# IDEA-CCNL/Fengshenbang-LM

Measured on AMD Instinct MI355X. Metric: tokens/sec Ziya-LLaMA-13B ZeRO-3, higher is better.
Workload: dtype bf16; 1 GPU; model=Ziya-LLaMA-13B, global_batch=16, micro_batch=16, seq_len=2048, parallelism=zero3_dp1, activation_checkpointing=True, ckpt_skip_interval=4

## Files before the change

fengshen_amd/models/layers.py:

```python
from __future__ import annotations

import math
from typing import Callable, List, Optional

import torch
import torch.nn as nn
import torch.nn.init as init

from fengshen_amd.ops import functional as F_ops
from fengshen_amd.parallel import groups
from fengshen_amd.parallel.layers import (
    ColumnParallelLinear,
    RowParallelLinear,
    _init_partition,
    divide,
)
from fengshen_amd.parallel.mappings import (
    copy_to_tensor_model_parallel_region,
    gather_from_tensor_model_parallel_region,
)


def init_normal(std: float) -> Callable:
    def fn(tensor):
# ... 219 lines not shown

    def __init__(self, hidden_size: int, intermediate_size: Optional[int] = None,
                 multiple_of: int = 256, init_method=None,
                 output_init_method=None, dtype=None,
                 reduce_output: bool = True):
        super().__init__()
        self.reduce_output = reduce_output
        if intermediate_size is None:
            intermediate_size = int(2 * (4 * hidden_size) / 3)
            intermediate_size = multiple_of * (
                (intermediate_size + multiple_of - 1) // multiple_of)
        self.intermediate_size = intermediate_size
        init_method = init_method or init.xavier_normal_
        self.gate_up_proj = MergedColumnParallelLinear(
            hidden_size, [intermediate_size, intermediate_size], bias=False,
            init_method=init_method, dtype=dtype)
        self.down_proj = RowParallelLinear(
            intermediate_size, hidden_size, bias=False, input_is_parallel=True,
            init_method=output_init_method or init_method, dtype=dtype,
            reduce_output=reduce_output)

    def forward(self, x):
        packed = self.gate_up_proj(x)
        h = F_ops.swiglu(packed)
        return self.down_proj(h)


class ParallelTransformerLayer(nn.Module):

    def __init__(self, hidden_size: int, num_heads: int, *, causal: bool,
                 norm: str = "layernorm", norm_eps: float = 1e-5,
                 mlp_type: str = "gelu", ffn_hidden_size=None,
                 rotary: bool = False, rope_base: float = 10000.0,
                 max_positions: int = 4096,
                 attention_dropout: float = 0.0, hidden_dropout: float = 0.0,
                 bias: bool = True, init_method=None, output_init_method=None,
                 dtype=None, layer_idx: int = 0,
                 parallel_residual: bool = False):
        super().__init__()
        self.parallel_residual = parallel_residual
        self.input_norm = get_norm(norm, hidden_size, norm_eps, dtype)
        self.attention = ParallelAttention(
            hidden_size, num_heads, causal=causal, rotary=rotary,
            rope_base=rope_base, max_positions=max_positions,
            attention_dropout=attention_dropout, hidden_dropout=hidden_dropout,
            bias=bias, init_method=init_method,
            output_init_method=output_init_method, dtype=dtype,
            layer_idx=layer_idx, reduce_output=not parallel_residual)
        self.post_attention_norm = get_norm(norm, hidden_size, norm_eps, dtype)
        if mlp_type == "swiglu":
            self.mlp = LLaMAParallelMLP(
                hidden_size, ffn_hidden_size, init_method=init_method,
                output_init_method=output_init_method, dtype=dtype,
                reduce_output=not parallel_residual)
        else:
            self.mlp = ParallelMLP(
                hidden_size, ffn_hidden_size, bias=bias, init_method=init_method,
                output_init_method=output_init_method, dtype=dtype,
                reduce_output=not parallel_residual)
        self.hidden_dropout = hidden_dropout

    @staticmethod
    def _split_partial(out):
        if isinstance(out, tuple):
            return out[0], out[1]
        return out, None

    def forward(self, x, attention_mask=None, cache=None):
        if self.parallel_residual:
            from fengshen_amd.parallel.mappings import (
                reduce_from_tensor_model_parallel_region)
            ap, ab = self._split_partial(self.attention(
                self.input_norm(x), attention_mask=attention_mask,
                cache=cache))
            mp, mb = self._split_partial(
                self.mlp(self.post_attention_norm(x)))
            total = reduce_from_tensor_model_parallel_region(ap + mp)
            bias = None
            if ab is not None or mb is not None:
                bias = (ab if ab is not None else 0)                     + (mb if mb is not None else 0)
            return F_ops.bias_dropout_add(total, bias, x,
                                          self.hidden_dropout,
                                          self.training)
        residual = x
        h = self.input_norm(x)
        attn_out = self.attention(h, attention_mask=attention_mask, cache=cache)
        x = F_ops.bias_dropout_add(attn_out, None, residual,
                                   self.hidden_dropout, self.training)
        residual = x
        h = self.post_attention_norm(x)
        mlp_out = self.mlp(h)
        x = F_ops.bias_dropout_add(mlp_out, None, residual,
                                   self.hidden_dropout, self.training)
        return x


def parallel_lm_logits(hidden: torch.Tensor, word_embeddings_weight: torch.Tensor,
                       parallel_output: bool = True):
    input_parallel = copy_to_tensor_model_parallel_region(hidden)
    logits_parallel = torch.nn.functional.linear(
        input_parallel, word_embeddings_weight)
    if parallel_output:
        return logits_parallel
    return gather_from_tensor_model_parallel_region(logits_parallel)


class SinusoidalPositionalEmbedding(nn.Module):

    def __init__(self, dim: int, base: float = 10000.0):
        super().__init__()
        self.dim = dim
        self.base = base

    def forward(self, positions: torch.Tensor) -> torch.Tensor:
        half = self.dim // 2
        inv = 1.0 / (self.base ** (torch.arange(
            half, device=positions.device, dtype=torch.float32) / half))
        ang = positions.float()[..., None] * inv
        return torch.cat([ang.sin(), ang.cos()], dim=-1)


class AliBi(nn.Module):

    def __init__(self, num_heads: int, mp_size: int = 1, mp_rank: int = 0):
        super().__init__()
        self.num_heads = num_heads
        slopes = torch.tensor(self._slopes(num_heads))
        per = num_heads // mp_size
        self.register_buffer("slopes", slopes[mp_rank * per:(mp_rank + 1) * per],
                             persistent=False)
        self._cache = None

    @staticmethod
    def _slopes(n: int):
        def pow2(n):
            start = 2.0 ** (-(2.0 ** -(math.log2(n) - 3)))
            return [start * (start ** i) for i in range(n)]
        if math.log2(n).is_integer():
            return pow2(n)
        closest = 2 ** math.floor(math.log2(n))
        return pow2(closest) + AliBi._slopes(2 * closest)[0::2][: n - closest]

    def forward(self, sq: int, sk: int, device, dtype):
        if (self._cache is None or self._cache.shape[-1] < sk
                or self._cache.device != device):
            pos = torch.arange(sk, device=device, dtype=torch.float32)
            self._cache = self.slopes.to(device)[:, None, None] * \
                (pos[None, None, :] - pos[None, :, None])
        bias = self._cache[:, :sq, :sk] if self._cache.shape[1] >= sq else \
            self._cache[:, -sq:, :sk]
        return bias.to(dtype)


class SoftEmbedding(nn.Module):

    def __init__(self, wte: nn.Module, n_tokens: int = 10,
                 init_range: float = 0.5):
        super().__init__()
        self.wte = wte
        self.n_tokens = n_tokens
        dim = wte.weight.shape[1]
        self.soft_prompt = nn.Parameter(
            torch.empty(n_tokens, dim).uniform_(-init_range, init_range))

    def forward(self, input_ids: torch.Tensor) -> torch.Tensor:
        emb = self.wte(input_ids)
        b = emb.shape[0]
        prompt = self.soft_prompt.unsqueeze(0).expand(b, -1, -1).to(emb.dtype)
        return torch.cat([prompt, emb], dim=1)


class SpatialGatingUnit(nn.Module):

# ... 70 lines not shown
```

fengshen_amd/ops/build.py:

```python
from __future__ import annotations

import glob
import os
import shutil
import sys

_OPS_DIR = os.path.dirname(os.path.abspath(__file__))
_CSRC = os.path.join(_OPS_DIR, "csrc")
_BUILD_DIR = os.path.join(_OPS_DIR, "_build")
_TARGET = os.path.join(_OPS_DIR, "_C.so")


def sources():
    srcs = [os.path.join(_CSRC, "bindings.cpp"),
            os.path.join(_CSRC, "kernels.hip")]
    fa = os.path.join(_CSRC, "flash_attn.hip")
    if os.path.exists(fa):
        srcs.append(fa)
    return srcs


def needs_rebuild() -> bool:
    if not os.path.exists(_TARGET):
        return True
    t = os.path.getmtime(_TARGET)
    deps = sources() + glob.glob(os.path.join(_CSRC, "*.h"))
    return any(os.path.getmtime(s) > t for s in deps)


def build(force: bool = False, verbose: bool = True) -> str:
    os.environ.setdefault("PYTORCH_ROCM_ARCH", "gfx950")
    if not force and not needs_rebuild():
        if verbose:
            print(f"[fengshen_amd.ops.build] up to date: {_TARGET}")
        return _TARGET
    from torch.utils.cpp_extension import load

    os.makedirs(_BUILD_DIR, exist_ok=True)
    load(
        name="_C",
        sources=sources(),
        extra_cflags=["-O3", "-std=c++17"],
        extra_cuda_cflags=["-O3", "-std=c++17", "--offload-arch=gfx950",
                           "-ffast-math"],
        build_directory=_BUILD_DIR,
        verbose=verbose,
        is_python_module=False,
        keep_intermediates=True,
    )
    built = os.path.join(_BUILD_DIR, "_C.so")
    if not os.path.exists(built):
        cands = glob.glob(os.path.join(_BUILD_DIR, "_C*.so"))
        if not cands:
            raise RuntimeError(f"extension build produced no .so in {_BUILD_DIR}")
        built = cands[0]
    shutil.copy2(built, _TARGET)
    if verbose:
        print(f"[fengshen_amd.ops.build] built {_TARGET}")
    build_data_helpers(force=force, verbose=verbose)
    return _TARGET


_DATA_DIR = os.path.normpath(os.path.join(_OPS_DIR, "..", "data"))
_HELPERS_SRC = os.path.join(_DATA_DIR, "csrc", "helpers.cpp")
_HELPERS_TARGET = os.path.join(_DATA_DIR, "_helpers.so")


def build_data_helpers(force: bool = False, verbose: bool = True) -> str:
    if not force and os.path.exists(_HELPERS_TARGET) and \
            os.path.getmtime(_HELPERS_TARGET) > os.path.getmtime(_HELPERS_SRC):
        return _HELPERS_TARGET
    import subprocess
    import sysconfig

    import pybind11

    cmd = [
        "c++", "-O3", "-std=c++17", "-shared", "-fPIC",
        f"-I{pybind11.get_include()}",
        f"-I{sysconfig.get_paths()['include']}",
        _HELPERS_SRC, "-o", _HELPERS_TARGET,
    ]
    subprocess.check_call(cmd)
    if verbose:
        print(f"[fengshen_amd.ops.build] built {_HELPERS_TARGET}")
    return _HELPERS_TARGET


if __name__ == "__main__":
    build(force="--force" in sys.argv)
```

fengshen_amd/ops/csrc/bindings.cpp:

```cpp
#include <torch/extension.h>

#include <hip/hip_runtime.h>
#include <c10/hip/HIPStream.h>

#include <vector>

enum FsDtype { FS_F32 = 0, FS_BF16 = 1, FS_F16 = 2 };

static int fs_dtype(const at::Tensor& t) {
  switch (t.scalar_type()) {
    case at::kFloat: return FS_F32;
    case at::kBFloat16: return FS_BF16;
    case at::kHalf: return FS_F16;
    default: TORCH_CHECK(false, "unsupported dtype ", t.scalar_type());
  }
}

static hipStream_t cur_stream() {
  return c10::hip::getCurrentHIPStream().stream();
}

extern "C" {
void fs_rms_norm_fwd(const void*, const void*, void*, float*, int, int, float,
                     int, hipStream_t);
void fs_rms_norm_bwd(const void*, const void*, const void*, const float*,
                     void*, float*, int, int, int, hipStream_t);
void fs_layer_norm_fwd(const void*, const void*, const void*, void*, float*,
                       float*, int, int, float, int, hipStream_t);
void fs_layer_norm_bwd(const void*, const void*, const void*, const float*,
                       const float*, void*, float*, float*, int, int, int,
                       hipStream_t);
void fs_scaled_softmax_fwd(const void*, const unsigned char*, void*, float,
                           int, int, int, int, int, int, int, int,
                           hipStream_t);
void fs_scaled_softmax_bwd(const void*, const void*, void*, float, int, int,
                           int, hipStream_t);
void fs_rope(const void*, void*, const float*, const float*, long, int, int,
             int, int, int, hipStream_t);
void fs_swiglu_fwd(const void*, void*, long, int, int, hipStream_t);
void fs_swiglu_bwd(const void*, const void*, void*, long, int, int,
                   hipStream_t);
void fs_bias_gelu(const void*, const void*, const void*, void*, long, int, int,
                  int, hipStream_t);
void fs_fused_adamw(float*, const void*, float*, float*, void*, long, float,
                    float, float, float, float, int, int, int, hipStream_t);
void fs_flash_attn_fwd(const void*, const void*, const void*, void*, float*,
                       const int*, int, int, int, int, int, int, float,
                       float, unsigned long long, hipStream_t);
void fs_flash_attn_bwd(const void*, const void*, const void*, const void*,
                       const void*, const float*, void*, void*, void*, float*,
                       const int*, int, int, int, int, int, int, float,
                       float, unsigned long long, hipStream_t);
void fs_bf16_gemv(const void*, const void*, void*, int, int, int,
                  hipStream_t);
void fs_add_rms_norm(const void*, const void*, const void*, void*, void*,
                     int, int, float, hipStream_t);
void fs_decode_attn(const void*, void*, void*, const float*, const float*,
                    const void*, void*, int, int, int, int, float, int,
                    hipStream_t);
void fs_w8_gemv(const void*, const float*, const void*, void*, int, int, int,
                hipStream_t);
void fs_vocab_ce_fwd(const void*, const long*, float*, float*, float*,
                     long, int, int, int, hipStream_t);
void fs_vocab_ce_bwd(const void*, const long*, const float*, const float*,
                     const float*, void*, long, int, int, int, hipStream_t);
void fs_flash_attn_fwd_v3(const void*, const void*, const void*, void*,
                          float*, const int*, int, int, int, int, int, float,
                          float, unsigned long long, hipStream_t);
void fs_flash_attn_bwd_v3(const void*, const void*, const void*, const void*,
                          const void*, const float*, void*, void*, void*,
                          float*, const int*, int, int, int, int, int, float,
                          float, unsigned long long, hipStream_t);
void fs_flash_attn_fwd_v3_strided(const void*, const void*, const void*,
                                  void*, float*, const int*, const long*,
                                  const long*, int, int, int, int, int, float,
                                  float, unsigned long long, hipStream_t);
void fs_flash_attn_bwd_v3_strided(const void*, const void*, const void*,
                                  const void*, const void*, const float*,
                                  void*, void*, void*, float*, const int*,
                                  const long*, const long*, const long*,
                                  const long*, int, int, int, int, int, float,
                                  float, unsigned long long, hipStream_t);
void fs_rope_inplace(void*, void*, const float*, const float*, int, int, int,
                     int, long, long, long, int, int, int, hipStream_t);
}

static std::vector<at::Tensor> rms_norm_fwd(at::Tensor x, at::Tensor w,
                                            double eps) {
  TORCH_CHECK(x.is_contiguous() && w.is_contiguous());
  const int H = x.size(-1);
  TORCH_CHECK(H % 8 == 0, "hidden must be divisible by 8");
  const long rows = x.numel() / H;
  auto out = at::empty_like(x);
  auto invrms = at::empty({rows}, x.options().dtype(at::kFloat));
  fs_rms_norm_fwd(x.data_ptr(), w.data_ptr(), out.data_ptr(),
                  invrms.data_ptr<float>(), (int)rows, H, (float)eps,
                  fs_dtype(x), cur_stream());
  return {out, invrms};
}

static std::vector<at::Tensor> rms_norm_bwd(at::Tensor gy, at::Tensor x,
                                            at::Tensor w, at::Tensor invrms) {
  const int H = x.size(-1);
  const long rows = x.numel() / H;
  auto gx = at::empty_like(x);
  auto gw32 = at::zeros({H}, x.options().dtype(at::kFloat));
  fs_rms_norm_bwd(gy.data_ptr(), x.data_ptr(), w.data_ptr(),
                  invrms.data_ptr<float>(), gx.data_ptr(),
                  gw32.data_ptr<float>(), (int)rows, H, fs_dtype(x),
                  cur_stream());
  return {gx, gw32.to(w.scalar_type())};
}

static std::vector<at::Tensor> layer_norm_fwd(at::Tensor x, at::Tensor w,
                                              c10::optional<at::Tensor> b,
                                              double eps) {
  TORCH_CHECK(x.is_contiguous());
  const int H = x.size(-1);
  TORCH_CHECK(H % 8 == 0, "hidden must be divisible by 8");
  const long rows = x.numel() / H;
  auto out = at::empty_like(x);
  auto mean = at::empty({rows}, x.options().dtype(at::kFloat));
  auto invstd = at::empty({rows}, x.options().dtype(at::kFloat));
  fs_layer_norm_fwd(x.data_ptr(), w.data_ptr(),
                    b.has_value() ? b->data_ptr() : nullptr, out.data_ptr(),
                    mean.data_ptr<float>(), invstd.data_ptr<float>(),
                    (int)rows, H, (float)eps, fs_dtype(x), cur_stream());
  return {out, mean, invstd};
}

static std::vector<at::Tensor> layer_norm_bwd(at::Tensor gy, at::Tensor x,
                                              at::Tensor w, at::Tensor mean,
                                              at::Tensor invstd) {
  const int H = x.size(-1);
  const long rows = x.numel() / H;
  auto gx = at::empty_like(x);
  auto gw32 = at::zeros({H}, x.options().dtype(at::kFloat));
  auto gb32 = at::zeros({H}, x.options().dtype(at::kFloat));
  fs_layer_norm_bwd(gy.data_ptr(), x.data_ptr(), w.data_ptr(),
                    mean.data_ptr<float>(), invstd.data_ptr<float>(),
                    gx.data_ptr(), gw32.data_ptr<float>(),
                    gb32.data_ptr<float>(), (int)rows, H, fs_dtype(x),
                    cur_stream());
  return {gx, gw32.to(w.scalar_type()), gb32.to(w.scalar_type())};
}

static at::Tensor scaled_masked_softmax_fwd(at::Tensor x,
                                            c10::optional<at::Tensor> mask,
                                            double scale) {
  TORCH_CHECK(x.dim() == 4 && x.is_contiguous());
  const int sk = x.size(3), sq = x.size(2), np = x.size(1), b = x.size(0);
  auto out = at::empty_like(x);
  const unsigned char* mp = nullptr;
  at::Tensor m8;
  int mb = 1, mode = 0, mask_sq = 1;
  if (mask.has_value()) {
    m8 = mask->to(at::kByte).contiguous();
    TORCH_CHECK(m8.dim() == 4 && m8.size(3) == sk &&
                    (m8.size(2) == sq || m8.size(2) == 1),
                "mask must be [mb,1,sq|1,sk]");
    mb = m8.size(0);
    mask_sq = m8.size(2);
    TORCH_CHECK(mb == 1 || mb == b, "mask batch must be 1 or b");
    mp = m8.data_ptr<unsigned char>();
    mode = 1;
  }
  fs_scaled_softmax_fwd(x.data_ptr(), mp, out.data_ptr(), (float)scale,
                        b * np * sq, sk, sq, np, mb, mask_sq, mode,
                        fs_dtype(x), cur_stream());
  return out;
}

static at::Tensor scaled_causal_softmax_fwd(at::Tensor x, double scale) {
  TORCH_CHECK(x.dim() == 3 && x.is_contiguous());
  const int sk = x.size(2), sq = x.size(1), ab = x.size(0);
  TORCH_CHECK(sq == sk, "causal softmax needs sq == sk");
  auto out = at::empty_like(x);
  fs_scaled_softmax_fwd(x.data_ptr(), nullptr, out.data_ptr(), (float)scale,
                        ab * sq, sk, sq, 1, 1, sq, 2, fs_dtype(x),
                        cur_stream());
  return out;
}

static at::Tensor scaled_softmax_bwd(at::Tensor gy, at::Tensor y,
                                     double scale) {
  TORCH_CHECK(gy.is_contiguous() && y.is_contiguous());
  const int sk = y.size(-1);
  const long rows = y.numel() / sk;
  auto gx = at::empty_like(y);
  fs_scaled_softmax_bwd(gy.data_ptr(), y.data_ptr(), gx.data_ptr(),
                        (float)scale, (int)rows, sk, fs_dtype(y),
                        cur_stream());
  return gx;
}
// ... 346 lines not shown
  mod.def("add_rms_norm", &add_rms_norm);
  mod.def("flash_attn_fwd", &flash_attn_fwd);
  mod.def("vocab_ce_fwd", [](at::Tensor logits2d, at::Tensor targets,
                             int64_t vstart, int64_t vend) {
    TORCH_CHECK(logits2d.is_contiguous() && logits2d.dim() == 2
                && logits2d.scalar_type() == at::kBFloat16);
    TORCH_CHECK(targets.scalar_type() == at::kLong
                && targets.is_contiguous());
    const long n = logits2d.size(0);
    const int w = logits2d.size(1);
    TORCH_CHECK(w % 8 == 0, "vocab shard must be divisible by 8");
    auto opts = logits2d.options().dtype(at::kFloat);
    auto m = at::empty({n}, opts);
    auto z = at::empty({n}, opts);
    auto pred = at::empty({n}, opts);
    fs_vocab_ce_fwd(logits2d.data_ptr(), targets.data_ptr<long>(),
                    m.data_ptr<float>(), z.data_ptr<float>(),
                    pred.data_ptr<float>(), n, w, (int)vstart, (int)vend,
                    cur_stream());
    return std::vector<at::Tensor>{m, z, pred};
  });
  mod.def("vocab_ce_bwd", [](at::Tensor logits2d, at::Tensor targets,
                             at::Tensor m, at::Tensor z, at::Tensor gout,
                             int64_t vstart, int64_t vend) {
    const long n = logits2d.size(0);
    const int w = logits2d.size(1);
    auto dl = at::empty_like(logits2d);
    fs_vocab_ce_bwd(logits2d.data_ptr(), targets.data_ptr<long>(),
                    m.data_ptr<float>(), z.data_ptr<float>(),
                    gout.contiguous().data_ptr<float>(), dl.data_ptr(), n, w,
                    (int)vstart, (int)vend, cur_stream());
    return dl;
  });
  mod.def("flash_attn_bwd_v3", [](at::Tensor q, at::Tensor k, at::Tensor v,
                                  at::Tensor o, at::Tensor dout,
                                  at::Tensor lse, double scale, bool causal,
                                  c10::optional<at::Tensor> klens,
                                  double drop_p, int64_t seed) {
    const int b = q.size(0), h = q.size(1), s = q.size(2), d = q.size(3);
    TORCH_CHECK((d == 128 || d == 96 || d == 64) && s % 64 == 0);
    const int* klp = nullptr;
    if (klens.has_value()) klp = klens->data_ptr<int>();
    auto dq = at::empty_like(q);
    auto dk = at::empty_like(k);
    auto dv = at::empty_like(v);
    auto delta = at::empty({b, h, s}, q.options().dtype(at::kFloat));
    fs_flash_attn_bwd_v3(q.data_ptr(), k.data_ptr(), v.data_ptr(),
                         o.data_ptr(), dout.contiguous().data_ptr(),
                         lse.data_ptr<float>(), dq.data_ptr(), dk.data_ptr(),
                         dv.data_ptr(), delta.data_ptr<float>(), klp, b, h,
                         s, d, causal ? 1 : 0, (float)scale, (float)drop_p,
                         (unsigned long long)seed, cur_stream());
    return std::vector<at::Tensor>{dq, dk, dv};
  });
  mod.def("flash_attn_fwd_v3", [](at::Tensor q, at::Tensor k, at::Tensor v,
                                  double scale, bool causal,
                                  c10::optional<at::Tensor> klens,
                                  double drop_p, int64_t seed) {
    TORCH_CHECK(q.is_contiguous() && k.is_contiguous() && v.is_contiguous());
    TORCH_CHECK(q.scalar_type() == at::kBFloat16);
    const int b = q.size(0), h = q.size(1), s = q.size(2), d = q.size(3);
    TORCH_CHECK((d == 128 || d == 96 || d == 64) && s % 64 == 0 && s >= 64);
    TORCH_CHECK(k.size(2) == s, "v3 is self-attention (sq == sk)");
    const int* klp = nullptr;
    if (klens.has_value()) {
      TORCH_CHECK(klens->scalar_type() == at::kInt
                  && klens->numel() == b && klens->is_contiguous());
      klp = klens->data_ptr<int>();
    }
    auto o = at::empty_like(q);
    auto lse = at::empty({b, h, s}, q.options().dtype(at::kFloat));
    fs_flash_attn_fwd_v3(q.data_ptr(), k.data_ptr(), v.data_ptr(),
                         o.data_ptr(), lse.data_ptr<float>(), klp, b, h, s,
                         d, causal ? 1 : 0, (float)scale, (float)drop_p,
                         (unsigned long long)seed, cur_stream());
    return std::vector<at::Tensor>{o, lse};
  });
  mod.def("flash_attn_bwd", &flash_attn_bwd);
  mod.def("flash_attn_fwd_v3_strided", &flash_attn_fwd_v3_strided);
  mod.def("flash_attn_bwd_v3_strided", &flash_attn_bwd_v3_strided);
  mod.def("rope_inplace", &rope_inplace);
  mod.def("rms_norm_fwd", &rms_norm_fwd);
  mod.def("rms_norm_bwd", &rms_norm_bwd);
  mod.def("layer_norm_fwd", &layer_norm_fwd);
  mod.def("layer_norm_bwd", &layer_norm_bwd);
  mod.def("scaled_masked_softmax_fwd", &scaled_masked_softmax_fwd);
  mod.def("scaled_causal_softmax_fwd", &scaled_causal_softmax_fwd);
  mod.def("scaled_softmax_bwd", &scaled_softmax_bwd);
  mod.def("rope_fwd", &rope_fwd);
  mod.def("rope_bwd", &rope_bwd);
  mod.def("swiglu_fwd", &swiglu_fwd);
  mod.def("swiglu_bwd", &swiglu_bwd);
  mod.def("bias_gelu_fwd", &bias_gelu_fwd);
  mod.def("bias_gelu_bwd", &bias_gelu_bwd);
  mod.def("fused_adamw", &fused_adamw);
}
```

fengshen_amd/ops/functional.py:

```python
from __future__ import annotations

import math
from typing import Optional

import torch

from fengshen_amd.ops import use_hip, get_ext


def eager_scaled_masked_softmax(x: torch.Tensor, mask: Optional[torch.Tensor],
                                scale: float) -> torch.Tensor:
    y = x.float() * scale
    if mask is not None:
        y = y.masked_fill(mask.bool(), -10000.0)
    return torch.softmax(y, dim=-1).to(x.dtype)


def eager_scaled_causal_softmax(x: torch.Tensor, scale: float) -> torch.Tensor:
    sq, sk = x.shape[-2], x.shape[-1]
    y = x.float() * scale
    causal = torch.ones(sq, sk, dtype=torch.bool, device=x.device).triu(1)
    y = y.masked_fill(causal, -10000.0)
    return torch.softmax(y, dim=-1).to(x.dtype)


class _ScaledMaskedSoftmax(torch.autograd.Function):
    @staticmethod
    def forward(ctx, x, mask, scale):
        if use_hip(x):
            out = get_ext().scaled_masked_softmax_fwd(x.contiguous(), mask,
                                                      scale)
        else:
            out = eager_scaled_masked_softmax(x, mask, scale)
        ctx.save_for_backward(out)
        ctx.scale = scale
        return out

    @staticmethod
    def backward(ctx, grad_out):
        (out,) = ctx.saved_tensors
        if use_hip(out):
            grad_in = get_ext().scaled_softmax_bwd(grad_out.contiguous(), out,
                                                   ctx.scale)
        else:
            g = grad_out.float() * out.float()
            grad_in = ((g - out.float() * g.sum(dim=-1, keepdim=True))
                       * ctx.scale).to(out.dtype)
        return grad_in, None, None


class _ScaledCausalSoftmax(torch.autograd.Function):
    @staticmethod
    def forward(ctx, x, scale):
        if use_hip(x):
            out = get_ext().scaled_causal_softmax_fwd(x.contiguous(), scale)
        else:
            out = eager_scaled_causal_softmax(x, scale)
        ctx.save_for_backward(out)
        ctx.scale = scale
        return out

    @staticmethod
    def backward(ctx, grad_out):
        (out,) = ctx.saved_tensors
        if use_hip(out):
            grad_in = get_ext().scaled_softmax_bwd(grad_out.contiguous(), out,
                                                   ctx.scale)
        else:
            g = grad_out.float() * out.float()
            grad_in = ((g - out.float() * g.sum(dim=-1, keepdim=True))
                       * ctx.scale).to(out.dtype)
        return grad_in, None


def scaled_masked_softmax(x, mask, scale: float = 1.0):
    return _ScaledMaskedSoftmax.apply(x, mask, scale)


def scaled_causal_softmax(x, scale: float = 1.0):
    return _ScaledCausalSoftmax.apply(x, scale)


def eager_rms_norm(x: torch.Tensor, weight: torch.Tensor, eps: float):
    x32 = x.float()
    var = x32.pow(2).mean(-1, keepdim=True)
    y = x32 * torch.rsqrt(var + eps)
    return (weight.float() * y).to(x.dtype)


class _RMSNorm(torch.autograd.Function):
    @staticmethod
    def forward(ctx, x, weight, eps):
        if use_hip(x):
            x = x.contiguous()
            out, invrms = get_ext().rms_norm_fwd(x, weight, eps)
        else:
            x32 = x.float()
            var = x32.pow(2).mean(-1, keepdim=True)
            invrms = torch.rsqrt(var + eps)
            out = (x32 * invrms * weight.float()).to(x.dtype)
        ctx.save_for_backward(x, weight, invrms)
        return out

    @staticmethod
    def backward(ctx, grad_out):
        x, weight, invrms = ctx.saved_tensors
        if use_hip(x):
            gx, gw = get_ext().rms_norm_bwd(grad_out.contiguous(), x, weight,
                                            invrms)
            return gx, gw, None
        x32 = x.float()
        g32 = grad_out.float()
        w32 = weight.float()
        xhat = x32 * invrms
        gy_w = g32 * w32
        mean_term = (gy_w * xhat).mean(-1, keepdim=True)
        gx = (invrms * (gy_w - xhat * mean_term)).to(x.dtype)
        gw = (g32 * xhat).sum(dim=tuple(range(x.dim() - 1))).to(weight.dtype)
        return gx, gw, None


def rms_norm(x, weight, eps: float = 1e-6):
    return _RMSNorm.apply(x, weight, eps)


def eager_layer_norm(x, weight, bias, eps):
    return torch.nn.functional.layer_norm(
        x.float(), (x.shape[-1],), weight.float(),
        bias.float() if bias is not None else None, eps).to(x.dtype)


class _LayerNorm(torch.autograd.Function):
    @staticmethod
    def forward(ctx, x, weight, bias, eps):
        if use_hip(x):
            x = x.contiguous()
            out, mean, invstd = get_ext().layer_norm_fwd(x, weight, bias, eps)
            ctx.save_for_backward(x, weight, mean, invstd)
            ctx.has_bias = bias is not None
            return out
        ctx.eps = eps
        ctx.fallback = True
        x32 = x.float()
        mean = x32.mean(-1, keepdim=True)
        var = x32.var(-1, unbiased=False, keepdim=True)
        invstd = torch.rsqrt(var + eps)
        out = (x32 - mean) * invstd * weight.float()
        if bias is not None:
            out = out + bias.float()
        ctx.save_for_backward(x, weight, mean, invstd)
        ctx.has_bias = bias is not None
        return out.to(x.dtype)

    @staticmethod
    def backward(ctx, grad_out):
        x, weight, mean, invstd = ctx.saved_tensors
        if use_hip(x):
            gx, gw, gb = get_ext().layer_norm_bwd(
                grad_out.contiguous(), x, weight, mean, invstd)
            return gx, gw, (gb if ctx.has_bias else None), None
        x32 = x.float()
        g32 = grad_out.float()
        w32 = weight.float()
        xhat = (x32 - mean) * invstd
        gy_w = g32 * w32
        n = x.shape[-1]
        gx = (invstd * (gy_w - gy_w.mean(-1, keepdim=True)
                        - xhat * (gy_w * xhat).mean(-1, keepdim=True))).to(x.dtype)
        dims = tuple(range(x.dim() - 1))
        gw = (g32 * xhat).sum(dims).to(weight.dtype)
        gb = g32.sum(dims).to(weight.dtype) if ctx.has_bias else None
        return gx, gw, gb, None


def layer_norm(x, weight, bias=None, eps: float = 1e-5):
    return _LayerNorm.apply(x, weight, bias, eps)


def eager_gelu(x):
    return x * 0.5 * (1.0 + torch.tanh(0.79788456 * x * (1 + 0.044715 * x * x)))


class _BiasGelu(torch.autograd.Function):
    @staticmethod
    def forward(ctx, x, bias):
        ctx.save_for_backward(x, bias)
        if use_hip(x):
            return get_ext().bias_gelu_fwd(x, bias)
        y = x.float() + bias.float()
        return eager_gelu(y).to(x.dtype)

    @staticmethod
    def backward(ctx, grad_out):
        x, bias = ctx.saved_tensors
        if use_hip(x):
            gx = get_ext().bias_gelu_bwd(grad_out.contiguous(), x, bias)
        else:
            y = (x.float() + bias.float())
            t = torch.tanh(0.79788456 * y * (1 + 0.044715 * y * y))
            ff = 0.5 * y * ((1 - t * t) * (0.79788456 + 0.1070322243 * y * y)) \
                + 0.5 * (1 + t)
            gx = (ff * grad_out.float()).to(x.dtype)
        gb = gx.sum(dim=tuple(range(gx.dim() - 1))).to(bias.dtype)
        return gx, gb


# ... 183 lines not shown
```

Measured before the change: 10170 tokens/s.

## Fuse residual add with RMSNorm forward and backward in decoder layers

```diff
diff --git a/fengshen_amd/models/layers.py b/fengshen_amd/models/layers.py
--- a/fengshen_amd/models/layers.py
+++ b/fengshen_amd/models/layers.py
@@ -325,13 +325,25 @@
             return F_ops.bias_dropout_add(total, bias, x,
                                           self.hidden_dropout,
                                           self.training)
+        fused = (isinstance(self.input_norm, RMSNorm)
+                 and isinstance(self.post_attention_norm, RMSNorm)
+                 and (self.hidden_dropout == 0.0 or not self.training))
+        if fused:
+            residual, h = F_ops.residual_rms_norm(
+                x, None, self.input_norm.weight, self.input_norm.eps)
+        else:
+            residual = x
+            h = self.input_norm(x)
+        attn_out = self.attention(h, attention_mask=attention_mask, cache=cache)
+        if fused and torch.is_tensor(attn_out):
+            x, h = F_ops.residual_rms_norm(
+                residual, attn_out, self.post_attention_norm.weight,
+                self.post_attention_norm.eps)
+        else:
+            x = F_ops.bias_dropout_add(attn_out, None, residual,
+                                       self.hidden_dropout, self.training)
+            h = self.post_attention_norm(x)
         residual = x
-        h = self.input_norm(x)
-        attn_out = self.attention(h, attention_mask=attention_mask, cache=cache)
-        x = F_ops.bias_dropout_add(attn_out, None, residual,
-                                   self.hidden_dropout, self.training)
-        residual = x
-        h = self.post_attention_norm(x)
         mlp_out = self.mlp(h)
         x = F_ops.bias_dropout_add(mlp_out, None, residual,
                                    self.hidden_dropout, self.training)
diff --git a/fengshen_amd/ops/build.py b/fengshen_amd/ops/build.py
--- a/fengshen_amd/ops/build.py
+++ b/fengshen_amd/ops/build.py
@@ -13,7 +13,8 @@
 
 def sources():
     srcs = [os.path.join(_CSRC, "bindings.cpp"),
-            os.path.join(_CSRC, "kernels.hip")]
+            os.path.join(_CSRC, "kernels.hip"),
+            os.path.join(_CSRC, "fused_norm.hip")]
     fa = os.path.join(_CSRC, "flash_attn.hip")
     if os.path.exists(fa):
         srcs.append(fa)
diff --git a/fengshen_amd/ops/csrc/bindings.cpp b/fengshen_amd/ops/csrc/bindings.cpp
--- a/fengshen_amd/ops/csrc/bindings.cpp
+++ b/fengshen_amd/ops/csrc/bindings.cpp
@@ -3,6 +3,7 @@
 #include <hip/hip_runtime.h>
 #include <c10/hip/HIPStream.h>
 
+#include <string>
 #include <vector>
 
 enum FsDtype { FS_F32 = 0, FS_BF16 = 1, FS_F16 = 2 };
@@ -83,6 +84,13 @@
                                   float, unsigned long long, hipStream_t);
 void fs_rope_inplace(void*, void*, const float*, const float*, int, int, int,
                      int, long, long, long, int, int, int, hipStream_t);
+int fs_fused_norm_vectors(int);
+int fs_fused_norm_bwd_grid(int, int);
+void fs_res_rms_norm_fwd(const void*, const void*, const void*, void*, void*,
+                         float*, int, int, float, int, hipStream_t);
+void fs_res_rms_norm_bwd(const void*, const void*, const void*, const void*,
+                         const float*, void*, float*, void*, int, int, int,
+                         hipStream_t);
 }
 
 static std::vector<at::Tensor> rms_norm_fwd(at::Tensor x, at::Tensor w,
@@ -110,6 +118,69 @@
                   gw32.data_ptr<float>(), (int)rows, H, fs_dtype(x),
                   cur_stream());
   return {gx, gw32.to(w.scalar_type())};
+}
+
+static std::string fused_norm_branch(int64_t H) {
+  const int nv = fs_fused_norm_vectors((int)H);
+  return nv ? "reg" + std::to_string(nv) : std::string("lds");
+}
+
+static std::vector<at::Tensor> residual_rms_norm_fwd(
+    at::Tensor x, c10::optional<at::Tensor> delta, at::Tensor w, double eps) {
+  TORCH_CHECK(x.is_contiguous() && w.is_contiguous());
+  const int H = x.size(-1);
+  TORCH_CHECK(H % 8 == 0, "hidden must be divisible by 8");
+  TORCH_CHECK(w.numel() == H && w.scalar_type() == x.scalar_type());
+  const bool has_delta = delta.has_value();
+  if (has_delta)
+    TORCH_CHECK(delta->is_contiguous() && delta->sizes() == x.sizes() &&
+                delta->scalar_type() == x.scalar_type());
+  if (fs_fused_norm_vectors(H) == 0) {
+    at::Tensor sum = has_delta ? at::add(x, *delta) : x;
+    auto r = rms_norm_fwd(sum, w, eps);
+    return {sum, r[0], r[1]};
+  }
+  const long rows = x.numel() / H;
+  at::Tensor sum = has_delta ? at::empty_like(x) : x;
+  auto h = at::empty_like(x);
+  auto invrms = at::empty({rows}, x.options().dtype(at::kFloat));
+  fs_res_rms_norm_fwd(x.data_ptr(), has_delta ? delta->data_ptr() : nullptr,
+                      w.data_ptr(), has_delta ? sum.data_ptr() : nullptr,
+                      h.data_ptr(), invrms.data_ptr<float>(), (int)rows, H,
+                      (float)eps, fs_dtype(x), cur_stream());
+  return {sum, h, invrms};
+}
+
+static std::vector<at::Tensor> residual_rms_norm_bwd(
+    at::Tensor g_h, c10::optional<at::Tensor> g_res, at::Tensor x,
+    at::Tensor w, at::Tensor invrms) {
+  TORCH_CHECK(g_h.is_contiguous() && x.is_contiguous() && w.is_contiguous());
+  TORCH_CHECK(g_h.sizes() == x.sizes() &&
+              g_h.scalar_type() == x.scalar_type());
+  const int H = x.size(-1);
+  const long rows = x.numel() / H;
+  TORCH_CHECK(H % 8 == 0, "hidden must be divisible by 8");
+  TORCH_CHECK(invrms.is_contiguous() && invrms.scalar_type() == at::kFloat &&
+              invrms.numel() == rows, "invrms must be ", rows, " floats");
+  TORCH_CHECK(w.numel() == H);
+  const bool has_res = g_res.has_value();
+  if (has_res)
+    TORCH_CHECK(g_res->is_contiguous() && g_res->sizes() == x.sizes() &&
+                g_res->scalar_type() == x.scalar_type());
+  if (fs_fused_norm_vectors(H) == 0) {
+    auto r = rms_norm_bwd(g_h, x, w, invrms);
+    return {has_res ? at::add(r[0], *g_res) : r[0], r[1]};
+  }
+  TORCH_CHECK(w.scalar_type() == x.scalar_type());
+  auto g = at::empty_like(x);
+  auto gw = at::empty_like(w);
+  auto part = at::empty({fs_fused_norm_bwd_grid((int)rows, H), H},
+                        x.options().dtype(at::kFloat));
+  fs_res_rms_norm_bwd(g_h.data_ptr(), has_res ? g_res->data_ptr() : nullptr,
+                      x.data_ptr(), w.data_ptr(), invrms.data_ptr<float>(),
+                      g.data_ptr(), part.data_ptr<float>(), gw.data_ptr(),
+                      (int)rows, H, fs_dtype(x), cur_stream());
+  return {g, gw};
 }
 
 static std::vector<at::Tensor> layer_norm_fwd(at::Tensor x, at::Tensor w,
@@ -622,6 +693,9 @@
   mod.def("rope_inplace", &rope_inplace);
   mod.def("rms_norm_fwd", &rms_norm_fwd);
   mod.def("rms_norm_bwd", &rms_norm_bwd);
+  mod.def("residual_rms_norm_fwd", &residual_rms_norm_fwd);
+  mod.def("residual_rms_norm_bwd", &residual_rms_norm_bwd);
+  mod.def("fused_norm_branch", &fused_norm_branch);
   mod.def("layer_norm_fwd", &layer_norm_fwd);
   mod.def("layer_norm_bwd", &layer_norm_bwd);
   mod.def("scaled_masked_softmax_fwd", &scaled_masked_softmax_fwd);
diff --git a/fengshen_amd/ops/csrc/fused_norm.hip b/fengshen_amd/ops/csrc/fused_norm.hip
--- /dev/null
+++ b/fengshen_amd/ops/csrc/fused_norm.hip
@@ -0,0 +1,351 @@
+
+#include "common.h"
+
+enum FsDtype { FS_F32 = 0, FS_BF16 = 1, FS_F16 = 2 };
+
+namespace {
+
+template <typename T>
+__device__ __forceinline__ float round_to(float v) {
+  return to_f32<T>(from_f32<T>(v));
+}
+
+constexpr int FN_THREADS = 256;
+constexpr int FN_WAVES = FN_THREADS / WAVE_SIZE;
+
+__device__ __forceinline__ float fn_block_sum(float v, float* red) {
+#pragma clang fp reassociate(off)
+  v = wave_reduce_sum(v);
+  if ((threadIdx.x & (WAVE_SIZE - 1)) == 0) red[threadIdx.x / WAVE_SIZE] = v;
+  __syncthreads();
+  const float a = red[0] + red[2];
+  const float b = red[1] + red[3];
+  return a + b;
+}
+
+__device__ __forceinline__ float row_partial(float acc, const float (&a)[8],
+                                             const float (&b)[8]) {
+#pragma clang fp reassociate(off) contract(off)
+  float lo = a[6] * b[6];
+  float hi = a[7] * b[7];
+  lo = __builtin_fmaf(a[2], b[2], lo);
+  hi = __builtin_fmaf(a[3], b[3], hi);
+  lo = __builtin_fmaf(a[4], b[4], lo);
+  hi = __builtin_fmaf(a[5], b[5], hi);
+  lo = __builtin_fmaf(a[0], b[0], lo);
+  hi = __builtin_fmaf(a[1], b[1], hi);
+  const float s = lo + hi;
+  return acc + s;
+}
+
+__device__ __forceinline__ float norm_out(float x, float ir, float w) {
+#pragma clang fp reassociate(off)
+  return (w * ir) * x;
+}
+
+__device__ __forceinline__ float norm_grad(float gyw, float xh, float dot,
+                                           float ir) {
+#pragma clang fp reassociate(off) contract(off)
+  return __builtin_fmaf(-dot, xh, gyw) * ir;
+}
+
+template <typename T>
+__device__ __forceinline__ float add_rounded(float inner, float r) {
+  float t = round_to<T>(inner);
+  if constexpr (sizeof(T) == 4) asm volatile("" : "+v"(t));
+  return t + r;
+}
+
+__device__ __forceinline__ float row_mean(float sum, int H) {
+#pragma clang fp reassociate(off)
+  return sum / H;
+}
+
+__device__ __forceinline__ void zero8(float (&v)[8]) {
+#pragma unroll
+  for (int i = 0; i < 8; ++i) v[i] = 0.f;
+}
+
+template <typename T> struct raw8 { short8_t v; };
+template <> struct raw8<float> { float4_t lo, hi; };
+
+template <typename T>
+__device__ __forceinline__ raw8<T> raw_zero() {
+  raw8<T> r;
+  r.v = short8_t{0, 0, 0, 0, 0, 0, 0, 0};
+  return r;
+}
+template <>
+__device__ __forceinline__ raw8<float> raw_zero<float>() {
+  raw8<float> r;
+  r.lo = float4_t{0.f, 0.f, 0.f, 0.f};
+  r.hi = r.lo;
+  return r;
+}
+
+template <typename T>
+__device__ __forceinline__ raw8<T> raw_load(const T* p) {
+  raw8<T> r;
+  r.v = *reinterpret_cast<const short8_t*>(p);
+  return r;
+}
+template <>
+__device__ __forceinline__ raw8<float> raw_load<float>(const float* p) {
+  raw8<float> r;
+  r.lo = reinterpret_cast<const float4_t*>(p)[0];
+  r.hi = reinterpret_cast<const float4_t*>(p)[1];
+  return r;
+}
+
+template <typename T>
+__device__ __forceinline__ void unpack8(const raw8<T>& r, float (&out)[8]) {
+  load8<T>(reinterpret_cast<const T*>(&r.v), out);
+}
+template <>
+__device__ __forceinline__ void unpack8<float>(const raw8<float>& r,
+                                               float (&out)[8]) {
+#pragma unroll
+  for (int i = 0; i < 4; ++i) { out[i] = r.lo[i]; out[4 + i] = r.hi[i]; }
+}
+
+template <typename T, int V, bool HAS_DELTA>
+__global__ __launch_bounds__(FN_THREADS) void res_rms_norm_fwd_kernel(
+    const T* __restrict__ x, const T* __restrict__ delta,
+    const T* __restrict__ w, T* __restrict__ sum_out, T* __restrict__ h_out,
+    float* __restrict__ invrms, int rows, int H, float eps) {
+  __shared__ float red[2][FN_WAVES];
+  int c[V];
+  bool act[V];
+  raw8<T> wr[V], xr[V], dr[V];
+  int row = blockIdx.x;
+#pragma unroll
+  for (int p = 0; p < V; ++p) {
+    c[p] = (threadIdx.x + p * FN_THREADS) * 8;
+    act[p] = c[p] < H;
+    wr[p] = xr[p] = dr[p] = raw_zero<T>();
+    if (act[p]) {
+      wr[p] = raw_load<T>(w + c[p]);
+      if (row < rows) {
+        xr[p] = raw_load<T>(x + (long)row * H + c[p]);
+        if (HAS_DELTA) dr[p] = raw_load<T>(delta + (long)row * H + c[p]);
+      }
+    }
+  }
+  int buf = 0;
+  for (; row < rows; row += gridDim.x) {
+    float v[V][8];
+#pragma unroll
+    for (int p = 0; p < V; ++p) {
+      unpack8<T>(xr[p], v[p]);
+      if (HAS_DELTA) {
+        float dv[8];
+        unpack8<T>(dr[p], dv);
+#pragma unroll
+        for (int i = 0; i < 8; ++i) v[p][i] = round_to<T>(v[p][i] + dv[i]);
+      }
+    }
+    const int nrow = row + gridDim.x;
+    if (nrow < rows) {
+#pragma unroll
+      for (int p = 0; p < V; ++p)
+        if (act[p]) {
+          xr[p] = raw_load<T>(x + (long)nrow * H + c[p]);
+          if (HAS_DELTA) dr[p] = raw_load<T>(delta + (long)nrow * H + c[p]);
+        }
+    }
+    float ss = 0.f;
+#pragma unroll
+    for (int p = 0; p < V; ++p) {
+      if (HAS_DELTA && act[p]) store8<T>(sum_out + (long)row * H + c[p], v[p]);
+      ss = row_partial(ss, v[p], v[p]);
+    }
+    ss = fn_block_sum(ss, red[buf]);
+    buf ^= 1;
+    const float ir = rsqrtf(ss / H + eps);
+    if (threadIdx.x == 0) invrms[row] = ir;
+#pragma unroll
+    for (int p = 0; p < V; ++p)
+      if (act[p]) {
+        float wv[8], o[8];
+        unpack8<T>(wr[p], wv);
+#pragma unroll
+        for (int i = 0; i < 8; ++i) o[i] = norm_out(v[p][i], ir, wv[i]);
+        store8<T>(h_out + (long)row * H + c[p], o);
+      }
+  }
+}
+
+template <typename T, int V, bool HAS_RES>
+__global__ __launch_bounds__(FN_THREADS) void res_rms_norm_bwd_kernel(
+    const T* __restrict__ gh, const T* __restrict__ gres,
+    const T* __restrict__ x, const T* __restrict__ w,
+    const float* __restrict__ invrms, T* __restrict__ g_out,
+    float* __restrict__ gw_part, int rows, int H) {
+  __shared__ float red[2][FN_WAVES];
+  int c[V];
+  bool act[V];
+  float acc[V][8];
+  raw8<T> wr[V], xr[V], gr[V], rr[V];
+  int row = blockIdx.x;
+#pragma unroll
+  for (int p = 0; p < V; ++p) {
+    c[p] = (threadIdx.x + p * FN_THREADS) * 8;
+    act[p] = c[p] < H;
+    zero8(acc[p]);
+    wr[p] = xr[p] = gr[p] = rr[p] = raw_zero<T>();
+    if (act[p]) {
+      wr[p] = raw_load<T>(w + c[p]);
+      if (row < rows) {
+        xr[p] = raw_load<T>(x + (long)row * H + c[p]);
+        gr[p] = raw_load<T>(gh + (long)row * H + c[p]);
+        if (HAS_RES) rr[p] = raw_load<T>(gres + (long)row * H + c[p]);
+      }
+    }
+  }
+  int buf = 0;
+  for (; row < rows; row += gridDim.x) {
+    const float ir = invrms[row];
+    float xh[V][8], gyw[V][8];
+    raw8<T> rcur[V];
+    float dot = 0.f;
+#pragma unroll
+    for (int p = 0; p < V; ++p) {
+      float xv[8], gv[8], wv[8];
+      unpack8<T>(xr[p], xv);
+      unpack8<T>(gr[p], gv);
+      unpack8<T>(wr[p], wv);
+#pragma unroll
+      for (int i = 0; i < 8; ++i) {
+        xh[p][i] = xv[i] * ir;
+        gyw[p][i] = gv[i] * wv[i];
+        acc[p][i] += gv[i] * xh[p][i];
+      }
+      dot = row_partial(dot, gyw[p], xh[p]);
+      rcur[p] = rr[p];
+    }
+    const int nrow = row + gridDim.x;
+    if (nrow < rows) {
+#pragma unroll
+      for (int p = 0; p < V; ++p)
+        if (act[p]) {
+          xr[p] = raw_load<T>(x + (long)nrow * H + c[p]);
+          gr[p] = raw_load<T>(gh + (long)nrow * H + c[p]);
+          if (HAS_RES) rr[p] = raw_load<T>(gres + (long)nrow * H + c[p]);
+        }
+    }
+    dot = row_mean(fn_block_sum(dot, red[buf]), H);
+    buf ^= 1;
+#pragma unroll
+    for (int p = 0; p < V; ++p)
+      if (act[p]) {
+        float o[8], r[8];
+        unpack8<T>(rcur[p], r);
+#pragma unroll
+        for (int i = 0; i < 8; ++i) {
+          o[i] = norm_grad(gyw[p][i], xh[p][i], dot, ir);
+          if (HAS_RES) o[i] = add_rounded<T>(o[i], r[i]);
+        }
+        store8<T>(g_out + (long)row * H + c[p], o);
+      }
+  }
+#pragma unroll
+  for (int p = 0; p < V; ++p)
+    if (act[p]) {
+      float4_t* q =
+          reinterpret_cast<float4_t*>(gw_part + (long)blockIdx.x * H + c[p]);
+      float4_t lo = {acc[p][0], acc[p][1], acc[p][2], acc[p][3]};
+      float4_t hi = {acc[p][4], acc[p][5], acc[p][6], acc[p][7]};
+      q[0] = lo;
+      q[1] = hi;
+    }
+}
+
+template <typename T>
+__global__ __launch_bounds__(512) void rms_norm_gw_reduce_kernel(
+    const float* __restrict__ part, T* __restrict__ gw, int P, int H) {
+  __shared__ float sm[8][64];
+  const int tx = threadIdx.x & 63;
+  const int ty = threadIdx.x >> 6;
+  const int col = blockIdx.x * 64 + tx;
+  float s = 0.f;
+  if (col < H)
+    for (int p = ty; p < P; p += 8) s += part[(long)p * H + col];
+  sm[ty][tx] = s;
+  __syncthreads();
+  if (ty == 0 && col < H) {
+    float t = 0.f;
+#pragma unroll
+    for (int i = 0; i < 8; ++i) t += sm[i][tx];
+    gw[col] = from_f32<T>(t);
+  }
+}
+
+#define FN_DISPATCH_DTYPE(dtype, T, ...)                      \
+  switch (dtype) {                                            \
+    case FS_F32: { using T = float; __VA_ARGS__; break; }     \
+    case FS_BF16: { using T = bf16_t; __VA_ARGS__; break; }   \
+    case FS_F16: { using T = fp16_t; __VA_ARGS__; break; }    \
+  }
+
+#define FN_DISPATCH_V(nv, V, ...)                             \
+  switch (nv) {                                               \
+    case 1: { constexpr int V = 1; __VA_ARGS__; break; }      \
+    case 2: { constexpr int V = 2; __VA_ARGS__; break; }      \
+    case 3: { constexpr int V = 3; __VA_ARGS__; break; }      \
+    case 4: { constexpr int V = 4; __VA_ARGS__; break; }      \
+  }
+
+#define FN_DISPATCH_BOOL(flag, B, ...)                        \
+  if (flag) { constexpr bool B = true; __VA_ARGS__; }         \
+  else { constexpr bool B = false; __VA_ARGS__; }
+
+}
+
+extern "C" {
+
+int fs_fused_norm_vectors(int H) {
+  if (H % 8 != 0 || H < 256 || H > 8192) return 0;
+  return (H + FN_THREADS * 8 - 1) / (FN_THREADS * 8);
+}
+
+int fs_fused_norm_bwd_grid(int rows, int H) {
+  if (fs_fused_norm_vectors(H) == 0) return 0;
+  const int g = rows < 1024 ? rows : 1024;
+  return g < 1 ? 1 : g;
+}
+
+void fs_res_rms_norm_fwd(const void* x, const void* delta, const void* w,
+                         void* sum_out, void* h_out, float* invrms, int rows,
+                         int H, float eps, int dtype, hipStream_t s) {
+  const int nv = fs_fused_norm_vectors(H);
+  int grid = rows < FS_MAX_BLOCKS ? rows : FS_MAX_BLOCKS;
+  if (grid < 1) grid = 1;
+  FN_DISPATCH_DTYPE(dtype, T,
+    FN_DISPATCH_V(nv, V,
+      FN_DISPATCH_BOOL(delta != nullptr, HD,
+        hipLaunchKernelGGL((res_rms_norm_fwd_kernel<T, V, HD>), dim3(grid),
+                           dim3(FN_THREADS), 0, s, (const T*)x,
+                           (const T*)delta, (const T*)w, (T*)sum_out,
+                           (T*)h_out, invrms, rows, H, eps))));
+}
+
+void fs_res_rms_norm_bwd(const void* gh, const void* gres, const void* x,
+                         const void* w, const float* invrms, void* g_out,
+                         float* gw_part, void* gw, int rows, int H, int dtype,
+                         hipStream_t s) {
+  const int nv = fs_fused_norm_vectors(H);
+  const int grid = fs_fused_norm_bwd_grid(rows, H);
+  FN_DISPATCH_DTYPE(dtype, T,
+    FN_DISPATCH_V(nv, V,
+      FN_DISPATCH_BOOL(gres != nullptr, HR,
+        hipLaunchKernelGGL((res_rms_norm_bwd_kernel<T, V, HR>), dim3(grid),
+                           dim3(FN_THREADS), 0, s, (const T*)gh,
+                           (const T*)gres, (const T*)x, (const T*)w, invrms,
+                           (T*)g_out, gw_part, rows, H))));
+  FN_DISPATCH_DTYPE(dtype, T,
+    hipLaunchKernelGGL((rms_norm_gw_reduce_kernel<T>), dim3((H + 63) / 64),
+                       dim3(512), 0, s, (const float*)gw_part, (T*)gw, grid,
+                       H));
+}
+
+}
diff --git a/fengshen_amd/ops/functional.py b/fengshen_amd/ops/functional.py
--- a/fengshen_amd/ops/functional.py
+++ b/fengshen_amd/ops/functional.py
@@ -1,6 +1,7 @@
 from __future__ import annotations
 
 import math
+import os
 from typing import Optional
 
 import torch
@@ -88,12 +89,33 @@
     return (weight.float() * y).to(x.dtype)
 
 
+def fused_norm_enabled() -> bool:
+    return os.environ.get("FENGSHEN_FUSED_NORM", "1") != "0"
+
+
+def _rms_norm_bwd_eager(g_h, x, weight, invrms):
+    x32 = x.float()
+    g32 = g_h.float()
+    w32 = weight.float()
+    xhat = x32 * invrms
+    gy_w = g32 * w32
+    mean_term = (gy_w * xhat).mean(-1, keepdim=True)
+    gx = (invrms * (gy_w - xhat * mean_term)).to(x.dtype)
+    gw = (g32 * xhat).sum(dim=tuple(range(x.dim() - 1))).to(weight.dtype)
+    return gx, gw
+
+
 class _RMSNorm(torch.autograd.Function):
     @staticmethod
     def forward(ctx, x, weight, eps):
+        ctx.fused = fused_norm_enabled()
         if use_hip(x):
             x = x.contiguous()
-            out, invrms = get_ext().rms_norm_fwd(x, weight, eps)
+            if ctx.fused:
+                _, out, invrms = get_ext().residual_rms_norm_fwd(
+                    x, None, weight, eps)
+            else:
+                out, invrms = get_ext().rms_norm_fwd(x, weight, eps)
         else:
             x32 = x.float()
             var = x32.pow(2).mean(-1, keepdim=True)
@@ -106,22 +128,64 @@
     def backward(ctx, grad_out):
         x, weight, invrms = ctx.saved_tensors
         if use_hip(x):
-            gx, gw = get_ext().rms_norm_bwd(grad_out.contiguous(), x, weight,
-                                            invrms)
+            if ctx.fused:
+                gx, gw = get_ext().residual_rms_norm_bwd(
+                    grad_out.contiguous(), None, x, weight, invrms)
+            else:
+                gx, gw = get_ext().rms_norm_bwd(grad_out.contiguous(), x,
+                                                weight, invrms)
             return gx, gw, None
-        x32 = x.float()
-        g32 = grad_out.float()
-        w32 = weight.float()
-        xhat = x32 * invrms
-        gy_w = g32 * w32
-        mean_term = (gy_w * xhat).mean(-1, keepdim=True)
-        gx = (invrms * (gy_w - xhat * mean_term)).to(x.dtype)
-        gw = (g32 * xhat).sum(dim=tuple(range(x.dim() - 1))).to(weight.dtype)
+        gx, gw = _rms_norm_bwd_eager(grad_out, x, weight, invrms)
         return gx, gw, None
 
 
 def rms_norm(x, weight, eps: float = 1e-6):
     return _RMSNorm.apply(x, weight, eps)
+
+
+class _ResidualRMSNorm(torch.autograd.Function):
+
+    @staticmethod
+    def forward(ctx, x, delta, weight, eps):
+        ctx.set_materialize_grads(False)
+        ctx.has_delta = delta is not None
+        if use_hip(x):
+            xc = x.contiguous()
+            dc = delta.contiguous() if ctx.has_delta else None
+            res, h, invrms = get_ext().residual_rms_norm_fwd(
+                xc, dc, weight, eps)
+            if not ctx.has_delta:
+                res = x
+        else:
+            res = x + delta if ctx.has_delta else x
+            r32 = res.float()
+            invrms = torch.rsqrt(r32.pow(2).mean(-1, keepdim=True) + eps)
+            h = (r32 * invrms * weight.float()).to(x.dtype)
+        ctx.save_for_backward(res, weight, invrms)
+        return res, h
+
+    @staticmethod
+    def backward(ctx, g_res, g_h):
+        res, weight, invrms = ctx.saved_tensors
+        if g_h is None:
+            g, gw = g_res, None
+        elif use_hip(res):
+            g, gw = get_ext().residual_rms_norm_bwd(
+                g_h.contiguous(), None if g_res is None else g_res.contiguous(),
+                res.contiguous(), weight, invrms)
+        else:
+            g, gw = _rms_norm_bwd_eager(g_h, res, weight, invrms)
+            if g_res is not None:
+                g = g + g_res
+        return g, (g if ctx.has_delta else None), gw, None
+
+
+def residual_rms_norm(x, delta, weight, eps: float = 1e-6):
+    if not fused_norm_enabled():
+        res = x if delta is None else bias_dropout_add(delta, None, x, 0.0,
+                                                       False)
+        return res, rms_norm(res, weight, eps)
+    return _ResidualRMSNorm.apply(x, delta, weight, eps)
 
 
 def eager_layer_norm(x, weight, bias, eps):
```

Result: faster. 10360 tokens/s, median of 6 (+1.8%).
